# tensorboy/centerpose

Hardware: AMD Instinct MI355X
Metric: images/sec end-to-end (backbone+decode), DLA-34 512x512 (higher is better)
Workload: dtype f32

## Files before the change

### centerpose_amd/csrc/head_wino24.hip

```cpp
#include "igemm.h"

#define HW_THREADS 512
#define HW_PH 18
#define HW_PW 18
#define HW_PWP 20
#define HW_C 64
#define HW_CGS (HW_C / 4)
#define HW_CG (HW_PH * HW_PWP * 4)
#define HW_PATCH (HW_CGS * HW_CG)
#define HW_F4 (HW_PH * HW_PW * HW_CGS)
#define HW_SLOTS ((HW_F4 + HW_THREADS - 1) / HW_THREADS)
#define HW_LDR 36
#define HW_RED (16 * 32 * HW_LDR)
#define HW_LDM 36
#define HW_MID (256 * HW_LDM)
#define HW_SMEM_FLOATS (2 * HW_RED)
#define HW_SMEM_FLOATS_MM (HW_RED + HW_MID > HW_PATCH ? HW_RED + HW_MID : HW_PATCH)

typedef float hw_v2 __attribute__((ext_vector_type(2)));
typedef float hw_v4 __attribute__((ext_vector_type(4)));

struct HwHead {
    const float* w2;
    const float* b2;
    float* out2;
    int n2, ld2, act2;
};
struct HwGrid {
    int tilesX, tilesY;
    unsigned mTx, mTy;
};
__device__ __forceinline__ hw_v4 hw_lds4(const float* p) { return *reinterpret_cast<const hw_v4*>(p); }
__device__ __forceinline__ int hw_div(int n, int d, unsigned magic) { return d == 1 ? n : (int)__umulhi((unsigned)n, magic); }

__device__ __forceinline__ void hw_write_share(const f32x16 (&acc)[3], const int vh, const int P, float* wq)
{
#pragma unroll
    for (int j = 0; j < 4; ++j) {
        hw_v4 q[3];
#pragma unroll
        for (int nu = 0; nu < 3; ++nu) q[nu] = (hw_v4){acc[nu][4 * j], acc[nu][4 * j + 1], acc[nu][4 * j + 2], acc[nu][4 * j + 3]};
        hw_v4 c0, c1;
        if (vh == 0) {
            const hw_v4 s1 = q[1] + q[2], d1 = q[1] - q[2];
            c0 = P == 0 ? q[0] + s1 : s1;
            c1 = d1;
        } else {
            const hw_v4 s2 = q[0] + q[1], d2 = q[0] - q[1];
            c0 = P == 0 ? s2 : 4.f * s2;
            c1 = P == 0 ? 2.f * d2 : 8.f * d2 + q[2];
        }
        *reinterpret_cast<hw_v4*>(wq + 8 * j) = c0;
        *reinterpret_cast<hw_v4*>(wq + 32 * HW_LDR + 8 * j) = c1;
    }
}

template <int N2, int MM, bool STAG>
__global__ __launch_bounds__(HW_THREADS, 1) void head_wino24_kernel(const ConvArgs a, const HwGrid gd, const HwHead hd)
{
    static_assert(!(STAG && MM), "the second-MFMA-phase form has no staggered variant");
    extern __shared__ __attribute__((aligned(16))) float smem[];
    const int tid = threadIdx.x, lane = tid & 63, wv = __builtin_amdgcn_readfirstlane(tid >> 6);
    const int xi = wv & 3, vh = wv >> 2;
    const int h = lane >> 5, m = lane & 31;
    const int NTILES = (a.Cout + 31) >> 5;
    int t_ = ig_xcd_remap(blockIdx.x, gridDim.x), q_;
    q_ = hw_div(t_, gd.tilesX, gd.mTx); const int tx = t_ - q_ * gd.tilesX; t_ = q_;
    q_ = hw_div(t_, gd.tilesY, gd.mTy); const int ty = t_ - q_ * gd.tilesY;
    const int b = q_;
    const int y0 = ty * 16, x0 = tx * 16;
    const int ld = a.srcLd[0];
    const float* __restrict__ x = a.src[0];

    {
        float4 rg[HW_SLOTS];
        int lo[HW_SLOTS];
        bool ok[HW_SLOTS];
#pragma unroll
        for (int s = 0; s < HW_SLOTS; ++s) {
            const int idx = tid + s * HW_THREADS;
            const int pp = idx / HW_CGS, q = idx % HW_CGS;
            const int py = pp / HW_PW, px = pp - py * HW_PW;
            const int gy = y0 - 1 + py, gx = x0 - 1 + px;
            const bool inl = idx < HW_F4;
            ok[s] = inl && gy >= 0 && gy < a.H && gx >= 0 && gx < a.W;
            const int go = ok[s] ? ((b * a.H + gy) * a.W + gx) * ld + q * 4 : 0;
            lo[s] = inl ? ((q * HW_PH + py) * HW_PWP + (px ^ ((py >> 1) & 3))) * 4 : -1;
            rg[s] = ig_ldg4(x + go);
        }
#pragma unroll
        for (int s = 0; s < HW_SLOTS; ++s)
            if (lo[s] >= 0) {
                float4 v = rg[s];
                if (!ok[s]) v = make_float4(0.f, 0.f, 0.f, 0.f);
                *reinterpret_cast<float4*>(smem + lo[s]) = v;
            }
    }
    const float* up = a.w + ((size_t)xi * NTILES * (HW_C / 8)) * 1536 + (size_t)(3 * vh) * 256 + lane * 4;
    const int nlin = NTILES * (HW_C / 8);
    float4 bq[2][3];
#pragma unroll
    for (int nu = 0; nu < 3; ++nu) bq[0][nu] = ig_ldg4(up + nu * 256);
    __syncthreads();
    if constexpr (STAG) {
        if (vh == 1) __syncthreads();
    }

    const int rA = xi == 0 ? 0 : (xi == 2 ? 2 : 1);
    const int rB = xi == 2 ? 1 : (xi == 3 ? 3 : 2);
    const float sg1 = xi == 1 ? 1.f : -1.f;
    const hw_v2 sg = {sg1, sg1};
    const int tyy = m >> 2, txx = m & 3;
    const int sA = (tyy + (rA >> 1)) & 3, sB = (tyy + (rB >> 1)) & 3;
    const int baseA = ((2 * tyy + rA) * HW_PWP + 4 * txx) * 4 + h * HW_CG;
    const int baseB = ((2 * tyy + rB) * HW_PWP + 4 * txx) * 4 + h * HW_CG;
    int offA[4], offB[4];
#pragma unroll
    for (int jj = 0; jj < 4; ++jj) { offA[jj] = baseA + ((jj ^ sA) << 2); offB[jj] = baseB + ((jj ^ sB) << 2); }
    hw_v2 vl[HW_C / 8][3], vhh[HW_C / 8][3];
#pragma unroll
    for (int kc = 0; kc < HW_C / 8; ++kc) {
        const float* pc = smem + kc * 2 * HW_CG;
        hw_v2 tl[5], th[5];
        if (vh == 0) {
#pragma unroll
            for (int j = 0; j < 5; ++j) {
                const hw_v4 da = hw_lds4(pc + offA[j & 3] + (j >> 2) * 16), db = hw_lds4(pc + offB[j & 3] + (j >> 2) * 16);
                tl[j] = __builtin_elementwise_fma(sg, db.xy, da.xy);
                th[j] = __builtin_elementwise_fma(sg, db.zw, da.zw);
            }
        } else {
#pragma unroll
            for (int j = 0; j < 5; ++j) {
                const int jc = j + 1;
                const hw_v4 da = hw_lds4(pc + offA[jc & 3] + (jc >> 2) * 16), db = hw_lds4(pc + offB[jc & 3] + (jc >> 2) * 16);
                tl[j] = __builtin_elementwise_fma(sg, db.xy, da.xy);
                th[j] = __builtin_elementwise_fma(sg, db.zw, da.zw);
            }
        }
        const hw_v2 k4 = {4.f, 4.f}, kn4 = {-4.f, -4.f}, k2 = {2.f, 2.f}, kn2 = {-2.f, -2.f};
        if (vh == 0) {
            const hw_v2 al = __builtin_elementwise_fma(kn4, tl[2], tl[4]), ah = __builtin_elementwise_fma(kn4, th[2], th[4]);
            const hw_v2 bl = __builtin_elementwise_fma(kn4, tl[1], tl[3]), bh = __builtin_elementwise_fma(kn4, th[1], th[3]);
            vl[kc][0] = __builtin_elementwise_fma(k4, tl[0] - tl[2], tl[4] - tl[2]); vhh[kc][0] = __builtin_elementwise_fma(k4, th[0] - th[2], th[4] - th[2]);
            vl[kc][1] = al + bl; vhh[kc][1] = ah + bh;
            vl[kc][2] = al - bl; vhh[kc][2] = ah - bh;
        } else {
            const hw_v2 cl = tl[3] - tl[1], ch = th[3] - th[1];
            const hw_v2 fl = tl[2] - tl[0], fh = th[2] - th[0];
            vl[kc][0] = __builtin_elementwise_fma(k2, fl, cl); vhh[kc][0] = __builtin_elementwise_fma(k2, fh, ch);
            vl[kc][1] = __builtin_elementwise_fma(kn2, fl, cl); vhh[kc][1] = __builtin_elementwise_fma(kn2, fh, ch);
            vl[kc][2] = __builtin_elementwise_fma(kn4, fl, tl[4] - tl[2]); vhh[kc][2] = __builtin_elementwise_fma(kn4, fh, th[4] - th[2]);
        }
#pragma unroll
        for (int nu = 0; nu < 3; ++nu) asm volatile("" : "+v"(vl[kc][nu]), "+v"(vhh[kc][nu]));
        __builtin_amdgcn_sched_barrier(0);
    }
    if constexpr (STAG) {
        if (vh == 0) __syncthreads();
    } else {
        __syncthreads();
    }

    float acc2[2][2][N2 > 0 ? N2 : 1];
#pragma unroll
    for (int i = 0; i < 2; ++i)
#pragma unroll
        for (int k = 0; k < 2; ++k)
#pragma unroll
            for (int j = 0; j < (N2 > 0 ? N2 : 1); ++j) acc2[i][k][j] = 0.f;
    f32x16 acc2m;
#pragma unroll
    for (int r = 0; r < 16; ++r) acc2m[r] = 0.f;
    constexpr int J0 = MM ? 32 : 0;
    float* const mid = smem + HW_RED;
    const int n4 = tid & 7, bb = (tid >> 3) & 1, mi = tid >> 4;
    const int ity = mi >> 2, itx = mi & 3;
    const int itrd = (bb * 32 + mi) * HW_LDR + n4 * 4;
    const int wpo = (wv * 64 + m) * HW_LDR + 4 * h;

    int lin = 0;
    if constexpr (!MM) {
        hw_v4 sc = {0.f, 0.f, 0.f, 0.f}, sh = sc, w2r[N2];
#pragma unroll
        for (int j = 0; j < N2; ++j) w2r[j] = sc;
        hw_v4 rq[8];
        auto red_read = [&](int P) __attribute__((always_inline)) {
            int rbase = itrd + P * HW_RED;
            asm volatile("" : "+v"(rbase));
            const float* rp = smem + rbase;
#pragma unroll
            for (int w = 0; w < 8; ++w) rq[w] = hw_lds4(rp + w * 64 * HW_LDR);
        };
        auto red_sum = [&](int P) __attribute__((always_inline)) {
            const hw_v4 r0 = rq[0] + rq[4], r1 = rq[1] + rq[5], r2 = rq[2] + rq[6], r3 = rq[3] + rq[7];
            hw_v4 yv[2];
            yv[0] = (r0 + r1) + r2;
            yv[1] = (r1 - r2) - r3;
#pragma unroll
            for (int aa = 0; aa < 2; ++aa) {
                hw_v4 v = __builtin_elementwise_fma(yv[aa], sc, sh);
                v = (hw_v4){cp_relu(v.x), cp_relu(v.y), cp_relu(v.z), cp_relu(v.w)};
#pragma unroll
                for (int j = 0; j < N2; ++j) {
                    const hw_v4 w = w2r[j];
                    acc2[P][aa][j] = fmaf(v.w, w.w, fmaf(v.z, w.z, fmaf(v.y, w.y, fmaf(v.x, w.x, acc2[P][aa][j]))));
                }
            }
        };
        if constexpr (STAG) {
            auto chunk = [&](const int kc, f32x16 (&acc)[3], auto&& ride) __attribute__((always_inline)) {
                ++lin;
                const float* un = up + (size_t)(lin < nlin ? lin : nlin - 1) * 1536;
                __builtin_amdgcn_sched_barrier(0);
#pragma unroll
                for (int nu = 0; nu < 3; ++nu) {
                    if (nu == 1) {
#pragma unroll
                        for (int q = 0; q < 3; ++q) bq[(kc + 1) & 1][q] = ig_ldg4(un + q * 256);
                        __builtin_amdgcn_sched_barrier(0);
                    }
                    if (nu == 2) {
                        ride();
                        __builtin_amdgcn_sched_barrier(0);
                    }
                    const float4 bbv = bq[kc & 1][nu];
                    acc[nu] = __builtin_amdgcn_mfma_f32_32x32x2f32(bbv.x, vl[kc][nu].x, acc[nu], 0, 0, 0);
                    acc[nu] = __builtin_amdgcn_mfma_f32_32x32x2f32(bbv.y, vl[kc][nu].y, acc[nu], 0, 0, 0);
                    acc[nu] = __builtin_amdgcn_mfma_f32_32x32x2f32(bbv.z, vhh[kc][nu].x, acc[nu], 0, 0, 0);
                    acc[nu] = __builtin_amdgcn_mfma_f32_32x32x2f32(bbv.w, vhh[kc][nu].y, acc[nu], 0, 0, 0);
                }
                __builtin_amdgcn_sched_barrier(0);
            };
            auto tile_end = [&](const int nt, const f32x16 (&acc)[3], const bool barrier_first) __attribute__((always_inline)) {
                const int ncol = nt * 32 + n4 * 4;
                sc = *reinterpret_cast<const hw_v4*>(a.scale + ncol);
                sh = *reinterpret_cast<const hw_v4*>(a.shift + ncol);
#pragma unroll
                for (int j = 0; j < N2; ++j) w2r[j] = *reinterpret_cast<const hw_v4*>(hd.w2 + (size_t)j * hd.ld2 + ncol);
                if (barrier_first) __syncthreads();
#pragma unroll
                for (int P = 0; P < 2; ++P) {
                    int wbase = wpo + P * HW_RED;
                    asm volatile("" : "+v"(wbase));
                    hw_write_share(acc, vh, P, smem + wbase);
                }
            };
            const auto nothing = [] {};
            if (vh == 0) {
#pragma unroll 1
                for (int nt = 0; nt < NTILES; ++nt) {
                    const bool prev = nt > 0;
                    f32x16 acc[3];
#pragma unroll
                    for (int nu = 0; nu < 3; ++nu)
#pragma unroll
                        for (int r = 0; r < 16; ++r) acc[nu][r] = 0.f;
#pragma unroll
                    for (int kc = 0; kc < 5; ++kc) chunk(kc, acc, nothing);
                    __syncthreads();
                    chunk(5, acc, [&] { if (prev) red_read(0); });
                    chunk(6, acc, [&] { if (prev) { red_sum(0); red_read(1); } });
                    chunk(7, acc, [&] { if (prev) red_sum(1); });
                    tile_end(nt, acc, true);
                }
            } else {
#pragma unroll 1
                for (int nt = 0; nt < NTILES; ++nt) {
                    const bool prev = nt > 0;
                    f32x16 acc[3];
#pragma unroll
                    for (int nu = 0; nu < 3; ++nu)
#pragma unroll
                        for (int r = 0; r < 16; ++r) acc[nu][r] = 0.f;
                    __syncthreads();
                    chunk(0, acc, [&] { if (prev) red_read(0); });
                    chunk(1, acc, [&] { if (prev) red_sum(0); });
                    chunk(2, acc, [&] { if (prev) red_read(1); });
                    chunk(3, acc, [&] { if (prev) red_sum(1); });
                    __syncthreads();
#pragma unroll
                    for (int kc = 4; kc < 8; ++kc) chunk(kc, acc, nothing);
                    tile_end(nt, acc, false);
                }
            }
            __syncthreads();
        } else {
#pragma unroll 1
        for (int nt = 0; nt < NTILES; ++nt) {
            const bool prev = nt > 0;
            f32x16 acc[3];
#pragma unroll
            for (int nu = 0; nu < 3; ++nu)
#pragma unroll
                for (int r = 0; r < 16; ++r) acc[nu][r] = 0.f;
#pragma unroll
            for (int kc = 0; kc < HW_C / 8; ++kc) {
                ++lin;
                const float* un = up + (size_t)(lin < nlin ? lin : nlin - 1) * 1536;
                __builtin_amdgcn_sched_barrier(0);
#pragma unroll
                for (int nu = 0; nu < 3; ++nu) {
                    if (nu == 1) {
#pragma unroll
                        for (int q = 0; q < 3; ++q) bq[(kc + 1) & 1][q] = ig_ldg4(un + q * 256);
                        __builtin_amdgcn_sched_barrier(0);
                    }
                    if (nu == 2 && prev) {
                        if (kc == 0) red_read(0);
                        if (kc == 2) red_sum(0);
                        if (kc == 4) red_read(1);
                        if (kc == 6) red_sum(1);
                        __builtin_amdgcn_sched_barrier(0);
                    }
                    const float4 bbv = bq[kc & 1][nu];
                    acc[nu] = __builtin_amdgcn_mfma_f32_32x32x2f32(bbv.x, vl[kc][nu].x, acc[nu], 0, 0, 0);
                    acc[nu] = __builtin_amdgcn_mfma_f32_32x32x2f32(bbv.y, vl[kc][nu].y, acc[nu], 0, 0, 0);
                    acc[nu] = __builtin_amdgcn_mfma_f32_32x32x2f32(bbv.z, vhh[kc][nu].x, acc[nu], 0, 0, 0);
                    acc[nu] = __builtin_amdgcn_mfma_f32_32x32x2f32(bbv.w, vhh[kc][nu].y, acc[nu], 0, 0, 0);
                }
                __builtin_amdgcn_sched_barrier(0);
            }
            const int ncol = nt * 32 + n4 * 4;
            sc = *reinterpret_cast<const hw_v4*>(a.scale + ncol);
            sh = *reinterpret_cast<const hw_v4*>(a.shift + ncol);
#pragma unroll
            for (int j = 0; j < N2; ++j) w2r[j] = *reinterpret_cast<const hw_v4*>(hd.w2 + (size_t)j * hd.ld2 + ncol);
            if (prev) __syncthreads();
#pragma unroll
            for (int P = 0; P < 2; ++P) {
                int wbase = wpo + P * HW_RED;
                asm volatile("" : "+v"(wbase));
                float* wq = smem + wbase;
#pragma unroll
                for (int j = 0; j < 4; ++j) {
                    hw_v4 q[3];
#pragma unroll
                    for (int nu = 0; nu < 3; ++nu) q[nu] = (hw_v4){acc[nu][4 * j], acc[nu][4 * j + 1], acc[nu][4 * j + 2], acc[nu][4 * j + 3]};
                    hw_v4 c0, c1;
                    if (vh == 0) {
                        const hw_v4 s1 = q[1] + q[2], d1 = q[1] - q[2];
                        c0 = P == 0 ? q[0] + s1 : s1;
                        c1 = d1;
                    } else {
                        const hw_v4 s2 = q[0] + q[1], d2 = q[0] - q[1];
                        c0 = P == 0 ? s2 : 4.f * s2;
                        c1 = P == 0 ? 2.f * d2 : 8.f * d2 + q[2];
                    }
                    *reinterpret_cast<hw_v4*>(wq + 8 * j) = c0;
                    *reinterpret_cast<hw_v4*>(wq + 32 * HW_LDR + 8 * j) = c1;
                }
            }
            __syncthreads();
        }
        }
        red_read(0); red_sum(0);
        red_read(1); red_sum(1);
    } else {
#pragma unroll 1
    for (int nt = 0; nt < NTILES; ++nt) {
        f32x16 acc[3];
#pragma unroll
        for (int nu = 0; nu < 3; ++nu)
#pragma unroll
            for (int r = 0; r < 16; ++r) acc[nu][r] = 0.f;
#pragma unroll
        for (int kc = 0; kc < HW_C / 8; ++kc) {
            ++lin;
            const float* un = up + (size_t)(lin < nlin ? lin : nlin - 1) * 1536;
            __builtin_amdgcn_sched_barrier(0);
#pragma unroll
            for (int nu = 0; nu < 3; ++nu) {
                if (nu == 1) {
#pragma unroll
                    for (int q = 0; q < 3; ++q) bq[(kc + 1) & 1][q] = ig_ldg4(un + q * 256);
                    __builtin_amdgcn_sched_barrier(0);
                }
                const float4 bbv = bq[kc & 1][nu];
                acc[nu] = __builtin_amdgcn_mfma_f32_32x32x2f32(bbv.x, vl[kc][nu].x, acc[nu], 0, 0, 0);
                acc[nu] = __builtin_amdgcn_mfma_f32_32x32x2f32(bbv.y, vl[kc][nu].y, acc[nu], 0, 0, 0);
                acc[nu] = __builtin_amdgcn_mfma_f32_32x32x2f32(bbv.z, vhh[kc][nu].x, acc[nu], 0, 0, 0);
                acc[nu] = __builtin_amdgcn_mfma_f32_32x32x2f32(bbv.w, vhh[kc][nu].y, acc[nu], 0, 0, 0);
            }
            __builtin_amdgcn_sched_barrier(0);
        }

        const int ncol = nt * 32 + n4 * 4;
        const hw_v4 sc = *reinterpret_cast<const hw_v4*>(a.scale + ncol), sh = *reinterpret_cast<const hw_v4*>(a.shift + ncol);
        hw_v4 w2r[N2 > 0 ? N2 : 1];
#pragma unroll
        for (int j = 0; j < N2; ++j) w2r[j] = *reinterpret_cast<const hw_v4*>(hd.w2 + (size_t)(J0 + j) * hd.ld2 + ncol);
        hw_v4 w2f[MM ? 4 : 1];
#pragma unroll
        for (int P = 0; P < 2; ++P) {
            if (MM && P == 1) __syncthreads();
            int wbase = wpo + (MM ? 0 : P * HW_RED), rbase = itrd + (MM ? 0 : P * HW_RED);
            asm volatile("" : "+v"(wbase), "+v"(rbase));
            float* wq = smem + wbase;
#pragma unroll
            for (int j = 0; j < 4; ++j) {
                hw_v4 q[3];
#pragma unroll
                for (int nu = 0; nu < 3; ++nu) q[nu] = (hw_v4){acc[nu][4 * j], acc[nu][4 * j + 1], acc[nu][4 * j + 2], acc[nu][4 * j + 3]};
                hw_v4 c0, c1;
                if (vh == 0) {
                    const hw_v4 s1 = q[1] + q[2], d1 = q[1] - q[2];
                    c0 = P == 0 ? q[0] + s1 : s1;
                    c1 = d1;
                } else {
                    const hw_v4 s2 = q[0] + q[1], d2 = q[0] - q[1];
                    c0 = P == 0 ? s2 : 4.f * s2;
                    c1 = P == 0 ? 2.f * d2 : 8.f * d2 + q[2];
                }
                *reinterpret_cast<hw_v4*>(wq + 8 * j) = c0;
                *reinterpret_cast<hw_v4*>(wq + 32 * HW_LDR + 8 * j) = c1;
            }
            if constexpr (MM) {
                if (P == 1) {
                    const int nmm = hd.n2 < 32 ? hd.n2 : 32;
                    const bool live = m < nmm;
                    const float* wrow = hd.w2 + (size_t)(live ? m : nmm - 1) * hd.ld2 + nt * 32 + 4 * h;
#pragma unroll
                    for (int s4 = 0; s4 < 4; ++s4) {
                        const float4 t4 = ig_ldg4(wrow + 8 * s4);
                        w2f[s4] = live ? (hw_v4){t4.x, t4.y, t4.z, t4.w} : (hw_v4){0.f, 0.f, 0.f, 0.f};
                    }
                }
            }
            __syncthreads();
            const float* rp = smem + rbase;
            hw_v4 r0 = hw_lds4(rp) + hw_lds4(rp + 4 * 64 * HW_LDR);
            const hw_v4 r1 = hw_lds4(rp + 64 * HW_LDR) + hw_lds4(rp + 5 * 64 * HW_LDR);
            const hw_v4 r2 = hw_lds4(rp + 2 * 64 * HW_LDR) + hw_lds4(rp + 6 * 64 * HW_LDR);
            const hw_v4 r3 = hw_lds4(rp + 3 * 64 * HW_LDR) + hw_lds4(rp + 7 * 64 * HW_LDR);
            hw_v4 yv[2];
            yv[0] = (r0 + r1) + r2;
            yv[1] = (r1 - r2) - r3;
#pragma unroll
            for (int aa = 0; aa < 2; ++aa) {
                hw_v4 v = __builtin_elementwise_fma(yv[aa], sc, sh);
                v = (hw_v4){cp_relu(v.x), cp_relu(v.y), cp_relu(v.z), cp_relu(v.w)};
#pragma unroll
                for (int j = 0; j < N2; ++j) {
                    const hw_v4 w = w2r[j];
                    acc2[P][aa][j] = fmaf(v.w, w.w, fmaf(v.z, w.z, fmaf(v.y, w.y, fmaf(v.x, w.x, acc2[P][aa][j]))));
                }
                if constexpr (MM) {
                    *reinterpret_cast<hw_v4*>(mid + ((2 * ity + aa) * 16 + 4 * itx + 2 * P + bb) * HW_LDM + n4 * 4) = v;
                }
            }
        }
        if constexpr (MM) {
            __syncthreads();
            const float* mp = mid + (32 * wv + m) * HW_LDM + 4 * h;
            hw_v4 mf[4];
#pragma unroll
            for (int s4 = 0; s4 < 4; ++s4) mf[s4] = hw_lds4(mp + 8 * s4);
#pragma unroll
            for (int s4 = 0; s4 < 4; ++s4) {
                acc2m = __builtin_amdgcn_mfma_f32_32x32x2f32(w2f[s4].x, mf[s4].x, acc2m, 0, 0, 0);
                acc2m = __builtin_amdgcn_mfma_f32_32x32x2f32(w2f[s4].y, mf[s4].y, acc2m, 0, 0, 0);
                acc2m = __builtin_amdgcn_mfma_f32_32x32x2f32(w2f[s4].z, mf[s4].z, acc2m, 0, 0, 0);
                acc2m = __builtin_amdgcn_mfma_f32_32x32x2f32(w2f[s4].w, mf[s4].w, acc2m, 0, 0, 0);
            }
            __syncthreads();
        }
    }

    }
    const size_t HW = (size_t)a.H * a.W;
    if constexpr (MM) {
        const int p = 32 * wv + m, ox = x0 + (p & 15), oy = y0 + (p >> 4);
        const int nmm = hd.n2 < 32 ? hd.n2 : 32;
        if (ox < a.W && oy < a.H) {
#pragma unroll
            for (int r = 0; r < 16; ++r) {
                const int j = (r & 3) + 8 * (r >> 2) + 4 * h;
                if (j < nmm) hd.out2[((size_t)b * hd.n2 + j) * HW + (size_t)oy * a.W + ox] = cp_act(acc2m[r] + hd.b2[j], hd.act2);
            }
        }
    }
    if constexpr (N2 > 0) {
#pragma unroll
        for (int P = 0; P < 2; ++P) {
            const int ox = x0 + 4 * itx + 2 * P + bb, oy = y0 + 2 * ity;
#pragma unroll
            for (int aa = 0; aa < 2; ++aa)
#pragma unroll
                for (int j = 0; j < N2; ++j) {
                    float v = acc2[P][aa][j];
                    v += __shfl_xor(v, 1);
                    v += __shfl_xor(v, 2);
                    v += __shfl_xor(v, 4);
                    if ((tid & 7) == 0 && J0 + j < hd.n2 && ox < a.W && oy + aa < a.H)
                        hd.out2[((size_t)b * hd.n2 + J0 + j) * HW + (size_t)(oy + aa) * a.W + ox] = cp_act(v + hd.b2[J0 + j], hd.act2);
                }
        }
    }
}

static unsigned hw_magic(int d) { return d <= 1 ? 0u : (unsigned)(((1ull << 32) + (unsigned)d - 1) / (unsigned)d); }

template <int N2, int MM, bool STAG = false>
static int launch_head_wino24(const ConvArgs& a, hipStream_t s, const HwHead& hd)
{
    const int smem = (MM ? HW_SMEM_FLOATS_MM : HW_SMEM_FLOATS) * 4;
    static CpLdsGuard guard;
    {
        const hipError_t e = guard.ensure((const void*)head_wino24_kernel<N2, MM, STAG>, smem);
        if (e != hipSuccess) { cp_set_error("head_wino24: cannot reserve %d B LDS: %s", smem, hipGetErrorString(e)); return 2; }
    }
    HwGrid gd;
    gd.tilesX = cp_cdiv(a.W, 16); gd.tilesY = cp_cdiv(a.H, 16);
    gd.mTx = hw_magic(gd.tilesX); gd.mTy = hw_magic(gd.tilesY);
    const long long grid = (long long)a.B * gd.tilesX * gd.tilesY;
    const long long dmax = gd.tilesX > gd.tilesY ? gd.tilesX : gd.tilesY;
    if (grid * dmax >= (1ll << 32)) { cp_set_error("head_wino24: grid %lld too large", grid); return 1; }
    hipLaunchKernelGGL((head_wino24_kernel<N2, MM, STAG>), dim3((unsigned)grid), dim3(HW_THREADS), smem, s, a, gd, hd);
    cp_note_kernel("head_wino24_kernel<%d, %d>", N2, MM);
    return 0;
}

int cp_launch_head3x3_1x1_w24(const ConvArgs& a, const float* w2, const float* b2, float* out2, int n2, int ld2, int act2, hipStream_t s)
{
    const bool ok = a.nsrc == 1 && a.kh == 3 && a.kw == 3 && a.sy == 1 && a.sx == 1 && a.py == 1 && a.px == 1 && a.Ho == a.H &&
                    a.Wo == a.W && a.srcC[0] == 64 && a.srcLd[0] % 4 == 0 && a.Cout % 32 == 0 && a.act == CP_ACT_RELU && !a.res &&
                    n2 >= 1 && n2 <= 34 && ld2 % 4 == 0 && ld2 >= a.Cout &&
                    (((size_t)a.src[0] | (size_t)a.w | (size_t)w2 | (size_t)a.scale | (size_t)a.shift) & 15) == 0 &&
                    (long long)a.B * a.H * a.W * a.srcLd[0] < (1ll << 31);
    if (!ok) return -1;
    HwHead hd;
    hd.w2 = w2; hd.b2 = b2; hd.out2 = out2; hd.n2 = n2; hd.ld2 = ld2; hd.act2 = act2;
    const char* sw = getenv("CP_HEAD_STAGGER");
    const bool stag = !(sw && sw[0] == '0');
    if (n2 == 1) return stag ? launch_head_wino24<1, 0, true>(a, s, hd) : launch_head_wino24<1, 0>(a, s, hd);
    if (n2 == 2) return stag ? launch_head_wino24<2, 0, true>(a, s, hd) : launch_head_wino24<2, 0>(a, s, hd);
    if (n2 <= 32) return launch_head_wino24<0, 1>(a, s, hd);
    if (n2 == 33) return launch_head_wino24<1, 1>(a, s, hd);
    return launch_head_wino24<2, 1>(a, s, hd);
}
```

### centerpose_amd/ops.py

```python
import ctypes
import os

import torch

from . import _lib

ACT_NONE, ACT_RELU, ACT_SIGMOID, ACT_HSWISH, ACT_HSIGMOID = 0, 1, 2, 3, 4
BN_EPS = 1e-5


class ConvDesc(ctypes.Structure):
    _fields_ = [(n, ctypes.c_int) for n in ("nsrc",)] + [("srcC", ctypes.c_int * 4), ("srcLd", ctypes.c_int * 4)] + \
        [(n, ctypes.c_int) for n in ("B", "H", "W", "Ho", "Wo", "kh", "kw", "sy", "sx", "py", "px", "K", "ldw", "Cout",
                                     "resLd", "outLd", "outNCHW", "OH", "OW", "osy", "osx", "ooy", "oox", "act",
                                     "inNCHW", "tile", "nsub", "ksplit")]


class DcnDesc(ctypes.Structure):
    _fields_ = [(n, ctypes.c_int) for n in ("B", "H", "W", "C", "srcLd", "Ho", "Wo", "kh", "kw", "sy", "sx", "py", "px",
                                            "dily", "dilx", "K", "ldw", "Cout", "omLd", "omSigmoid", "outLd",
                                            "outNCHW", "act", "tile", "ksplit", "dg")]


def round_up(x, m):
# ... 154 lines not shown


BATCH_INVARIANT = os.environ.get("CP_BATCH_INVARIANT", "0") == "1"


def rule_batch(B):
    return 1 if BATCH_INVARIANT else B


SPLIT_BF16 = os.environ.get("CP_SPLIT_BF16", "0") == "1"
SPLIT_BF16_TILES = ((128, 128), (128, 64), (64, 128), (64, 64))


def split_bf16_weight(wp, ldw):
    L = _lib.lib()
    rows, K = wp.shape
    assert rows % ldw == 0 and K % 16 == 0 and wp.is_contiguous()
    L.cp_split_bf16_weight_floats.restype = ctypes.c_size_t
    wb = torch.empty((L.cp_split_bf16_weight_floats(rows, K),), dtype=torch.float32, device=wp.device)
    _lib.check(L.cp_split_bf16_weights_f32(_lib.ptr(wp), rows, ldw, K, _lib.ptr(wb), _lib.stream()), "cp_split_bf16_weights_f32")
    return wb


def split_bf16_tile(M, ldw, nsub=1, ksplit=1, force=False, K=None):
    if ldw % 64:
        return None
    code = lambda bm, bn: 3000000 + bm * 1000 + bn
    forced = os.environ.get("CP_SPLIT_BF16_TILE")
    if forced:
        bm, bn = (int(v) for v in forced.split("x")) if "x" in forced else (128, int(forced))
        return code(bm, bn if ldw % bn == 0 else 64)
    blocks = lambda bm, bn: ((M + bm - 1) // bm) * max(1, nsub) * max(1, ksplit) * (ldw // bn)
    floor = 0 if force else int(os.environ.get("CP_SPLIT_BF16_MINBLOCKS", "512"))
    if floor == 0:
        return code(128, 128) if ldw % 128 == 0 and blocks(128, 128) >= 256 else code(128, 64)
    if ksplit > 1:
        return None
    order = ((64, 64),) if K is not None and K <= 64 else ((128, 128), (64, 128), (64, 64))
    for bm, bn in order:
        if ldw % bn == 0 and blocks(bm, bn) >= floor:
            return code(bm, bn)
    return None


def conv2d(srcs, wp, scale, shift, out, **kw):
    conv2d_launch(srcs, wp, scale, shift, out, **kw).run()
    return out


def conv2d_launch(srcs, wp, scale, shift, out, *, kh, kw, stride=1, pad=0, cout, act=ACT_NONE, res=None, out_nchw=False,
                  in_nchw=False, Ho=None, Wo=None, pad_yx=None, out_scatter=None, tile=0, wino=None, nsub=1, ksplit=0, split_bf16=None):
    d = ConvDesc()
    d.nsrc = len(srcs)
    if in_nchw:
        x = srcs[0]
        B, C, H, W = x.shape
        d.srcC[0], d.srcLd[0] = C, 0
        assert B * C * H * W < 2 ** 31, "conv2d: NCHW source of %d floats exceeds the 32-bit element index of the stem producers" % (B * C * H * W)
        assert x.is_contiguous()
    else:
        B, H, W, _ = srcs[0].shape
        for i, s in enumerate(srcs):
            assert s.shape[:3] == srcs[0].shape[:3]
            d.srcC[i], d.srcLd[i] = s.shape[3], _ld(s)
    py, px = pad_yx if pad_yx is not None else (pad, pad)
    if Ho is None:
        Ho = (H + 2 * py - kh) // stride + 1
        Wo = (W + 2 * px - kw) // stride + 1
    assert B * Ho * Wo + 255 < 2 ** 31, "conv2d: B*Ho*Wo=%d output pixels exceed the 32-bit row index" % (B * Ho * Wo)
    d.B, d.H, d.W, d.Ho, d.Wo = B, H, W, Ho, Wo
    d.kh, d.kw, d.sy, d.sx, d.py, d.px = kh, kw, stride, stride, py, px
    assert wp.shape[0] % nsub == 0
    d.K, d.ldw, d.Cout, d.nsub = wp.shape[1], wp.shape[0] // nsub, cout, nsub
    d.resLd = _ld(res) if res is not None else 0
    d.outNCHW = 1 if out_nchw else 0
    d.ksplit = ksplit
    if ksplit > 1:
        assert res is None and act == ACT_NONE and not out_nchw and out.is_contiguous() and (wino is not None or (len(srcs) == 1 and not in_nchw and nsub == 1))
        assert tuple(out.shape[:2]) == (ksplit, B * Ho * Wo) and out.shape[2] >= cout and out.shape[2] % 4 == 0
        d.OH, d.OW, d.outLd = Ho, Wo, out.shape[2]
    elif out_nchw:
        d.OH, d.OW, d.outLd = out.shape[2], out.shape[3], 0
        assert out.is_contiguous() and out.shape[1] == cout
    else:
        d.OH, d.OW, d.outLd = out.shape[1], out.shape[2], _ld(out)
    d.osy, d.osx, d.ooy, d.oox = out_scatter if out_scatter is not None else (1, 1, 0, 0)
    d.act, d.inNCHW, d.tile = act, 1 if in_nchw else 0, tile
    for t in (wp, scale, shift, wino):
        assert t is None or t.is_contiguous()
    if wino is not None:
        assert len(srcs) == 1 and not in_nchw
        return Launch("cp_conv3x3_winograd_f32", d, [srcs[0], wino, scale, shift, res, out])
    if (SPLIT_BF16 if split_bf16 is None else split_bf16) and tile == 0 and not in_nchw:
        code = split_bf16_tile(rule_batch(B) * Ho * Wo, d.ldw, nsub, ksplit, force=split_bf16 is True, K=d.K)
        c16 = kh == 3 and kw == 3 and len(srcs) == 1 and srcs[0].shape[3] == 16 and cout <= 32
        if code is not None and not c16 and all(s.data_ptr() % 16 == 0 for s in srcs):
            d.tile = code
            wp = split_bf16_weight(wp, d.ldw)
    return Launch("cp_conv2d_f32", d, list(srcs) + [None] * (4 - len(srcs)) + [wp, scale, shift, res, out])


ConvDesc4 = ConvDesc * 4


def conv3x3_group_launch(members, whole):
    assert 1 <= len(members) <= 4
    members = sorted(members, key=lambda mm: -mm["x"].shape[3])
    d = ConvDesc4()
    cols = [[None] * 4 for _ in range(6)]
    for i, mm in enumerate(members):
        one = conv2d_launch([mm["x"]], mm["wp"], mm["scale"], mm["shift"], mm["out"], kh=3, kw=3, stride=1, pad=1, cout=mm["cout"],
                            act=mm["act"], res=mm["res"], wino=mm["u24"], tile=WINO24)
        ctypes.memmove(ctypes.addressof(d[i]), ctypes.addressof(one.desc), ctypes.sizeof(ConvDesc))
        for k, t in enumerate((mm["x"], mm["u24"], mm["scale"], mm["shift"], mm["res"], mm["out"])):
            cols[k][i] = t
            assert t is None or k in (0, 4, 5) or t.is_contiguous()
        assert mm["out"].untyped_storage().data_ptr() == whole.untyped_storage().data_ptr()
    return Launch("cp_conv3x3_winograd24_group_f32", d, [t for col in cols for t in col] + [whole], [len(members)])


ConvDesc8 = ConvDesc * 8
GROUP_MAX = 8


def conv2d_group_launch(members, whole):
    assert 1 <= len(members) <= GROUP_MAX
    members = sorted(members, key=lambda mm: -mm["wp"].shape[1])
    d = ConvDesc8()
    cols = [[None] * GROUP_MAX for _ in range(6)]
    for i, mm in enumerate(members):
        assert mm["wp"].shape[0] % 64 == 0
        one = conv2d_launch([mm["x"]], mm["wp"], mm["scale"], mm["shift"], mm["out"], kh=mm["k"], kw=mm["k"], stride=mm["stride"],
                            pad=mm["pad"], cout=mm["cout"], act=mm["act"], res=mm.get("res"), split_bf16=False)
        ctypes.memmove(ctypes.addressof(d[i]), ctypes.addressof(one.desc), ctypes.sizeof(ConvDesc))
        for k, t in enumerate((mm["x"], mm["wp"], mm["scale"], mm["shift"], mm.get("res"), mm["out"])):
            cols[k][i] = t
            assert t is None or k in (0, 4, 5) or t.is_contiguous()
        assert mm["out"].untyped_storage().data_ptr() == whole.untyped_storage().data_ptr()
    return Launch("cp_conv2d_group_f32", d, [t for col in cols for t in col] + [whole], [len(members)])


def head3x3_1x1_eligible(x, hc, n2):
    B, H, W, C = x.shape
    B = rule_batch(B)
    return C == 64 and hc % 32 == 0 and hc >= 128 and 1 <= n2 <= 34 and B * ((H + 7) // 8) * ((W + 15) // 16) >= 512


def head_wino24_wanted(x, n2):
    B, H, W, _ = x.shape
    B = rule_batch(B)
    mode = os.environ.get("CP_HEAD24", "1")
    if mode == "0" or B * ((H + 15) // 16) * ((W + 15) // 16) < 256:
        return False
    return mode == "all" or n2 <= 32


def head3x3_1x1_launch(x, u, scale, shift, w2, b2, out2, *, hc, act2=ACT_NONE, wino24=False):
    B, H, W, C = x.shape
    n2, ld2 = w2.shape
    assert out2.is_contiguous() and tuple(out2.shape) == (B, n2, H, W) and w2.is_contiguous() and b2.numel() >= n2
    d = ConvDesc()
    d.nsrc = 1
    d.srcC[0], d.srcLd[0] = C, _ld(x)
    d.B, d.H, d.W, d.Ho, d.Wo = B, H, W, H, W
    d.kh, d.kw, d.sy, d.sx, d.py, d.px = 3, 3, 1, 1, 1, 1
    d.K, d.ldw, d.Cout = 9 * C, round_up(hc, 64), hc
    d.resLd, d.outLd, d.outNCHW = 0, hc, 0
    d.OH, d.OW, d.osy, d.osx, d.ooy, d.oox = H, W, 1, 1, 0, 0
    d.act, d.inNCHW, d.tile, d.nsub = ACT_RELU, 0, WINO24 if wino24 else 0, 1
    return Launch("cp_head3x3_1x1_f32", d, [x, u, scale, shift, w2, b2, out2], [n2, ld2, act2])


def wino_eligible(cin, k, stride, pad, nsrc=1):
    return k == 3 and stride == 1 and pad == 1 and nsrc == 1 and cin % 16 == 0 and cin >= 32


def pack_wino_weight(wp, cin, cout):
    L = _lib.lib()
    assert wp.shape[1] == 9 * cin and wp.shape[0] >= cout and wp.is_contiguous()
    L.cp_winograd_weight_floats.restype = ctypes.c_size_t
    n = L.cp_winograd_weight_floats(cin, cout)
    assert n > 0, "winograd: C must be a multiple of 16"
    u = torch.empty((n,), dtype=torch.float32, device=wp.device)
    _lib.check(L.cp_winograd_pack_f32(_lib.ptr(wp), _lib.ptr(u), cin, cout, _lib.stream()), "cp_winograd_pack_f32")
    return u


def pack_wino24_weight(wp, cin, cout):
    L = _lib.lib()
    assert wp.shape[1] == 9 * cin and wp.shape[0] >= cout and wp.is_contiguous()
    L.cp_winograd24_weight_floats.restype = ctypes.c_size_t
    n = L.cp_winograd24_weight_floats(cin, cout)
    assert n > 0, "winograd: C must be a multiple of 16"
    u = torch.empty((n,), dtype=torch.float32, device=wp.device)
    _lib.check(L.cp_winograd24_pack_f32(_lib.ptr(wp), _lib.ptr(u), cin, cout, _lib.stream()), "cp_winograd24_pack_f32")
    return u


WINO24 = 24


def wino24_wanted(B, H, W, cin, cout):
    if os.environ.get("CP_WINO24", "1") == "0" or cin % 16 or cin < 32:
        return False
    minc, mincout, minblocks = (int(v) for v in os.environ.get("CP_WINO24_RULE", "32,16,256").split(","))
    blocks = rule_batch(B) * ((H + 15) // 16) * ((W + 15) // 16) * ((cout + 31) // 32)
    return cin >= minc and cout >= mincout and blocks >= minblocks


def dcn_v2(x, om, wp, scale, shift, out, **kw):
    dcn_v2_launch(x, om, wp, scale, shift, out, **kw).run()
    return out


def _pair(v):
    return (int(v[0]), int(v[1])) if isinstance(v, (tuple, list)) else (int(v), int(v))


def dcn_v2_launch(x, om, wp, scale, shift, out, *, cout, kh=3, kw=3, stride=1, pad=1, dil=1, om_sigmoid=True,
                  act=ACT_NONE, out_nchw=False, tile=0, ksplit=0, dg=1):
    B, H, W, C = x.shape
    d = DcnDesc()
    (sy, sx), (py, px), (dy, dx) = _pair(stride), _pair(pad), _pair(dil)
    Ho = (H + 2 * py - (dy * (kh - 1) + 1)) // sy + 1
    Wo = (W + 2 * px - (dx * (kw - 1) + 1)) // sx + 1
    assert om.shape[:3] == (B, Ho, Wo)
    d.B, d.H, d.W, d.C, d.srcLd, d.Ho, d.Wo = B, H, W, C, _ld(x), Ho, Wo
    d.kh, d.kw, d.sy, d.sx, d.py, d.px, d.dily, d.dilx = kh, kw, sy, sx, py, px, dy, dx
    d.K, d.ldw, d.Cout = wp.shape[1], wp.shape[0], cout
    d.omLd, d.omSigmoid = _ld(om), 1 if om_sigmoid else 0
    d.outNCHW = 1 if out_nchw else 0
    d.act, d.tile, d.ksplit, d.dg = act, tile, ksplit, dg
    if ksplit > 1:
        assert tuple(out.shape) == (ksplit, B * Ho * Wo, wp.shape[0]) and out.is_contiguous() and cout == wp.shape[0] and act == ACT_NONE
        d.outLd = wp.shape[0]
    else:
        d.outLd = 0 if out_nchw else _ld(out)
    return Launch("cp_dcn_v2_f32", d, [x, om, wp, scale, shift, out])


def wino_ksplit(B, H, W, cin, cout):
    blocks = rule_batch(B) * ((H + 7) // 8) * ((W + 15) // 16) * ((cout + 31) // 32)
    stages = cin // 16
    S = 1
    while blocks * S < 512 and stages // (2 * S) >= 4:
        S *= 2
    return S if blocks < 256 else 1


def conv_ksplit(M, ldw, K):
    if ldw % 64 != 0:
        return 1
    blocks = ((M + 63) // 64) * (ldw // 64)
    if blocks >= 400:
        return 1
    for S in (2, 3, 4):
        if blocks * S >= 512 and (K // 16) // S >= 16:
            return S
    return 1


def dcn_ksplit(M, ldw, taps=9):
    if ldw % 64 != 0 or taps < 3:
        return 1
    blocks = -(-M // 64) * (ldw // 64)
    return 3 if blocks < 512 else 1


def splitk_reduce_launch(ws, scale, shift, out, *, cout, act=ACT_NONE):
    S, M, ldw = ws.shape
    assert ws.is_contiguous() and out.shape[0] * out.shape[1] * out.shape[2] == M and scale.numel() >= ldw and shift.numel() >= ldw
    return Launch("cp_splitk_reduce_f32", None, [ws, scale, shift, out], [S, M, ldw, act, _ld(out), cout])


def maxpool2d_launch(x, out, k, s, p):
    B, H, W, C = x.shape
    return Launch("cp_maxpool2d_nhwc_f32", None, [x, out], [_ld(x), _ld(out), B, H, W, C, k, s, p])


def maxpool2d(x, out, k, s, p):
    maxpool2d_launch(x, out, k, s, p).run()
    return out


def pack_dw_deconv_weight(w):
    C, _, k, _ = w.shape
    return w.reshape(C, k * k).t().contiguous().float()


def dw_deconv_add_launch(x, wk, add, out, f):
    B, H, W, C = x.shape
    assert wk.is_contiguous()
    return Launch("cp_dw_deconv_add_nhwc_f32", None, [x, wk, add, out],
                  [_ld(x), _ld(add) if add is not None else 0, _ld(out), B, H, W, C, f])


def dw_deconv_add(x, wk, add, out, f):
    dw_deconv_add_launch(x, wk, add, out, f).run()
    return out


def pack_dw_weight(w):
    C, _, k, _ = w.shape
    return w.reshape(C, k * k).t().contiguous().float()


def dwconv2d_launch(x, wk, scale, shift, out, k, stride, pad, act=ACT_NONE):
# ... 214 lines not shown
```

Before: 2255.

## Add staggered two-group schedule for MFMA-phase Winograd head kernels and enable by default

Adds a staggered variant of the fused 3x3+1x1 Winograd head kernel for the second-MFMA-phase (n2>2) forms: the two wave groups run offset tile schedules, so one group's reduction, mid-tile write and 1x1 MFMA phase overlap the other group's main MFMA chunks. For n2==34, per-thread partial sums are parked in LDS to save registers. Wino24 is also enabled by default for heads with n2>32. This adds barriers and LDS traffic, and register pressure may still be a risk.

```diff
diff --git a/centerpose_amd/csrc/head_wino24.hip b/centerpose_amd/csrc/head_wino24.hip
--- a/centerpose_amd/csrc/head_wino24.hip
+++ b/centerpose_amd/csrc/head_wino24.hip
@@ -1,5 +1,9 @@
 #include "igemm.h"
-
+#include <type_traits>
+
+#ifndef HW_SETPRIO
+#define HW_SETPRIO 0
+#endif
 #define HW_THREADS 512
 #define HW_PH 18
 #define HW_PW 18
@@ -16,6 +20,8 @@
 #define HW_MID (256 * HW_LDM)
 #define HW_SMEM_FLOATS (2 * HW_RED)
 #define HW_SMEM_FLOATS_MM (HW_RED + HW_MID > HW_PATCH ? HW_RED + HW_MID : HW_PATCH)
+#define HW_PARK(N2, MM, STAG) ((N2) == 2 && (MM) && (STAG))
+#define HW_SMEM_FLOATS_PARK (2 * HW_RED + HW_THREADS * 8)
 
 typedef float hw_v2 __attribute__((ext_vector_type(2)));
 typedef float hw_v4 __attribute__((ext_vector_type(4)));
@@ -55,10 +61,36 @@
     }
 }
 
+template <class Ride>
+__device__ __forceinline__ void hw_chunk(const int kc, f32x16 (&acc)[3], float4 (&bq)[2][3], const hw_v2 (&vl)[HW_C / 8][3],
+                                         const hw_v2 (&vhh)[HW_C / 8][3], const float* up, int& lin, const int nlin, Ride&& ride)
+{
+    ++lin;
+    const float* un = up + (size_t)(lin < nlin ? lin : nlin - 1) * 1536;
+    __builtin_amdgcn_sched_barrier(0);
+#pragma unroll
+    for (int nu = 0; nu < 3; ++nu) {
+        if (nu == 1) {
+#pragma unroll
+            for (int q = 0; q < 3; ++q) bq[(kc + 1) & 1][q] = ig_ldg4(un + q * 256);
+            __builtin_amdgcn_sched_barrier(0);
+        }
+        if (nu == 2) {
+            ride();
+            __builtin_amdgcn_sched_barrier(0);
+        }
+        const float4 bbv = bq[kc & 1][nu];
+        acc[nu] = __builtin_amdgcn_mfma_f32_32x32x2f32(bbv.x, vl[kc][nu].x, acc[nu], 0, 0, 0);
+        acc[nu] = __builtin_amdgcn_mfma_f32_32x32x2f32(bbv.y, vl[kc][nu].y, acc[nu], 0, 0, 0);
+        acc[nu] = __builtin_amdgcn_mfma_f32_32x32x2f32(bbv.z, vhh[kc][nu].x, acc[nu], 0, 0, 0);
+        acc[nu] = __builtin_amdgcn_mfma_f32_32x32x2f32(bbv.w, vhh[kc][nu].y, acc[nu], 0, 0, 0);
+    }
+    __builtin_amdgcn_sched_barrier(0);
+}
+
 template <int N2, int MM, bool STAG>
 __global__ __launch_bounds__(HW_THREADS, 1) void head_wino24_kernel(const ConvArgs a, const HwGrid gd, const HwHead hd)
 {
-    static_assert(!(STAG && MM), "the second-MFMA-phase form has no staggered variant");
     extern __shared__ __attribute__((aligned(16))) float smem[];
     const int tid = threadIdx.x, lane = tid & 63, wv = __builtin_amdgcn_readfirstlane(tid >> 6);
     const int xi = wv & 3, vh = wv >> 2;
@@ -180,6 +212,7 @@
     const int wpo = (wv * 64 + m) * HW_LDR + 4 * h;
 
     int lin = 0;
+    int te = tid;
     if constexpr (!MM) {
         hw_v4 sc = {0.f, 0.f, 0.f, 0.f}, sh = sc, w2r[N2];
 #pragma unroll
@@ -210,27 +243,7 @@
         };
         if constexpr (STAG) {
             auto chunk = [&](const int kc, f32x16 (&acc)[3], auto&& ride) __attribute__((always_inline)) {
-                ++lin;
-                const float* un = up + (size_t)(lin < nlin ? lin : nlin - 1) * 1536;
-                __builtin_amdgcn_sched_barrier(0);
-#pragma unroll
-                for (int nu = 0; nu < 3; ++nu) {
-                    if (nu == 1) {
-#pragma unroll
-                        for (int q = 0; q < 3; ++q) bq[(kc + 1) & 1][q] = ig_ldg4(un + q * 256);
-                        __builtin_amdgcn_sched_barrier(0);
-                    }
-                    if (nu == 2) {
-                        ride();
-                        __builtin_amdgcn_sched_barrier(0);
-                    }
-                    const float4 bbv = bq[kc & 1][nu];
-                    acc[nu] = __builtin_amdgcn_mfma_f32_32x32x2f32(bbv.x, vl[kc][nu].x, acc[nu], 0, 0, 0);
-                    acc[nu] = __builtin_amdgcn_mfma_f32_32x32x2f32(bbv.y, vl[kc][nu].y, acc[nu], 0, 0, 0);
-                    acc[nu] = __builtin_amdgcn_mfma_f32_32x32x2f32(bbv.z, vhh[kc][nu].x, acc[nu], 0, 0, 0);
-                    acc[nu] = __builtin_amdgcn_mfma_f32_32x32x2f32(bbv.w, vhh[kc][nu].y, acc[nu], 0, 0, 0);
-                }
-                __builtin_amdgcn_sched_barrier(0);
+                hw_chunk(kc, acc, bq, vl, vhh, up, lin, nlin, ride);
             };
             auto tile_end = [&](const int nt, const f32x16 (&acc)[3], const bool barrier_first) __attribute__((always_inline)) {
                 const int ncol = nt * 32 + n4 * 4;
@@ -265,6 +278,9 @@
                     tile_end(nt, acc, true);
                 }
             } else {
+#if HW_SETPRIO
+                __builtin_amdgcn_s_setprio(1);
+#endif
 #pragma unroll 1
                 for (int nt = 0; nt < NTILES; ++nt) {
                     const bool prev = nt > 0;
@@ -356,6 +372,208 @@
         }
         red_read(0); red_sum(0);
         red_read(1); red_sum(1);
+    } else if constexpr (STAG) {
+        constexpr bool PARK = HW_PARK(N2, MM, STAG);
+        constexpr int NR = N2 > 0 ? N2 : 1;
+        hw_v4 sc, sh, w2r[NR], w2f[4], rq[4], r01[2], vm[2], mf[4];
+        const int nmm = hd.n2 < 32 ? hd.n2 : 32;
+        int o_rd, o_wp, o_mw, o_mp;
+        int o_a2;
+        unsigned wro, cbo;
+        bool live;
+        auto own_offsets = [&]() __attribute__((always_inline)) {
+            int t = tid;
+            asm volatile("" : "+v"(t));
+            const int tm = t & 31, th = (t >> 5) & 1, t4 = t & 7, tb = (t >> 3) & 1, ti = t >> 4;
+            o_rd = (tb * 32 + ti) * HW_LDR + t4 * 4;
+            o_wp = (wv * 64 + tm) * HW_LDR + 4 * th;
+            o_mw = (2 * (ti >> 2) * 16 + 4 * (ti & 3) + tb) * HW_LDM + t4 * 4;
+            o_mp = (32 * wv + tm) * HW_LDM + 4 * th;
+            live = tm < nmm;
+            wro = (unsigned)(((live ? tm : nmm - 1) * hd.ld2 + 4 * th) * 4);
+            cbo = (unsigned)(t4 * 16);
+            o_a2 = 2 * HW_RED + t * 8;
+            asm volatile("" : "+v"(o_a2));
+        };
+        auto gld = [](const float* base, const unsigned byteoff) __attribute__((always_inline)) {
+            asm volatile("" : "+s"(base));
+            return *(const __attribute__((address_space(1))) hw_v4*)(reinterpret_cast<const char*>(base) + byteoff);
+        };
+        auto cols_load = [&](const int pt) __attribute__((always_inline)) {
+            sc = gld(a.scale + pt * 32, cbo);
+            sh = gld(a.shift + pt * 32, cbo);
+#pragma unroll
+            for (int j = 0; j < N2; ++j) w2r[j] = gld(hd.w2 + (size_t)(J0 + j) * hd.ld2 + pt * 32, cbo);
+        };
+        auto w2f_load = [&](const int pt) __attribute__((always_inline)) {
+#pragma unroll
+            for (int s4 = 0; s4 < 4; ++s4) {
+                const hw_v4 t4 = gld(hd.w2 + pt * 32 + 8 * s4, wro);
+                w2f[s4] = live ? t4 : (hw_v4){0.f, 0.f, 0.f, 0.f};
+            }
+        };
+        auto red_read = [&](const int P) __attribute__((always_inline)) {
+            int rbase = o_rd + P * HW_RED;
+            asm volatile("" : "+v"(rbase));
+            const float* rp = smem + rbase;
+            rq[0] = hw_lds4(rp);                  rq[1] = hw_lds4(rp + 4 * 64 * HW_LDR);
+            rq[2] = hw_lds4(rp + 64 * HW_LDR);    rq[3] = hw_lds4(rp + 5 * 64 * HW_LDR);
+            r01[0] = rq[0] + rq[1];
+            r01[1] = rq[2] + rq[3];
+            __builtin_amdgcn_sched_barrier(0);
+            rq[0] = hw_lds4(rp + 2 * 64 * HW_LDR); rq[1] = hw_lds4(rp + 6 * 64 * HW_LDR);
+            rq[2] = hw_lds4(rp + 3 * 64 * HW_LDR); rq[3] = hw_lds4(rp + 7 * 64 * HW_LDR);
+        };
+        auto red_vals = [&](const int P) __attribute__((always_inline)) {
+            const hw_v4 r0 = r01[0], r1 = r01[1], r2 = rq[0] + rq[1], r3 = rq[2] + rq[3];
+            hw_v4 yv[2];
+            yv[0] = (r0 + r1) + r2;
+            yv[1] = (r1 - r2) - r3;
+#pragma unroll
+            for (int aa = 0; aa < 2; ++aa) {
+                hw_v4 v = __builtin_elementwise_fma(yv[aa], sc, sh);
+                v = (hw_v4){cp_relu(v.x), cp_relu(v.y), cp_relu(v.z), cp_relu(v.w)};
+#pragma unroll
+                for (int j = 0; j < N2; ++j) {
+                    const hw_v4 w = w2r[j];
+                    float* const park = smem + o_a2 + (P * 2 + aa) * N2 + j;
+                    const float s0 = PARK ? *park : acc2[P][aa][j];
+                    const float s1 = fmaf(v.w, w.w, fmaf(v.z, w.z, fmaf(v.y, w.y, fmaf(v.x, w.x, s0))));
+                    if constexpr (PARK) *park = s1;
+                    else acc2[P][aa][j] = s1;
+                }
+                vm[aa] = v;
+            }
+        };
+        auto mid_write = [&](const int P) __attribute__((always_inline)) {
+#pragma unroll
+            for (int aa = 0; aa < 2; ++aa) *reinterpret_cast<hw_v4*>(smem + o_mw + (aa * 16 + 2 * P) * HW_LDM) = vm[aa];
+        };
+        auto mid_read = [&]() __attribute__((always_inline)) {
+#pragma unroll
+            for (int s4 = 0; s4 < 4; ++s4) mf[s4] = hw_lds4(smem + o_mp + 8 * s4);
+        };
+        auto phase2 = [&]() __attribute__((always_inline)) {
+#pragma unroll
+            for (int s4 = 0; s4 < 4; ++s4) {
+                acc2m = __builtin_amdgcn_mfma_f32_32x32x2f32(w2f[s4].x, mf[s4].x, acc2m, 0, 0, 0);
+                acc2m = __builtin_amdgcn_mfma_f32_32x32x2f32(w2f[s4].y, mf[s4].y, acc2m, 0, 0, 0);
+                acc2m = __builtin_amdgcn_mfma_f32_32x32x2f32(w2f[s4].z, mf[s4].z, acc2m, 0, 0, 0);
+                acc2m = __builtin_amdgcn_mfma_f32_32x32x2f32(w2f[s4].w, mf[s4].w, acc2m, 0, 0, 0);
+            }
+        };
+        auto write_shares = [&](const f32x16 (&acc)[3]) __attribute__((always_inline)) {
+#pragma unroll
+            for (int P = 0; P < 2; ++P) {
+                int wbase = o_wp + P * HW_RED;
+                asm volatile("" : "+v"(wbase));
+                hw_write_share(acc, vh, P, smem + wbase);
+            }
+        };
+        auto chunk = [&](float4 (&bl)[2][3], const int kc, f32x16 (&acc)[3], auto&& ride) __attribute__((always_inline)) {
+            hw_chunk(kc, acc, bl, vl, vhh, up, lin, nlin, ride);
+        };
+        auto zero_sums = [&]() __attribute__((always_inline)) {
+#pragma unroll
+            for (int i = 0; i < 2; ++i)
+#pragma unroll
+                for (int k = 0; k < 2; ++k)
+#pragma unroll
+                    for (int j = 0; j < NR; ++j) {
+                        if constexpr (PARK) smem[o_a2 + (i * 2 + k) * N2 + j] = 0.f;
+                        else acc2[i][k][j] = 0.f;
+                    }
+#pragma unroll
+            for (int r = 0; r < 16; ++r) acc2m[r] = 0.f;
+        };
+        const auto nothing = [] {};
+        auto tile_a = [&](float4 (&bl)[2][3], const int nt, auto prev_c) __attribute__((always_inline)) {
+            constexpr bool PREV = decltype(prev_c)::value;
+            if constexpr (!PREV) { own_offsets(); zero_sums(); }
+            f32x16 acc[3];
+#pragma unroll
+            for (int nu = 0; nu < 3; ++nu)
+#pragma unroll
+                for (int r = 0; r < 16; ++r) acc[nu][r] = 0.f;
+#pragma unroll
+            for (int kc = 0; kc < 5; ++kc) chunk(bl, kc, acc, nothing);
+            __syncthreads();
+            chunk(bl, 5, acc, [&] { if constexpr (PREV) { cols_load(nt - 1); red_read(0); } });
+            chunk(bl, 6, acc, [&] { if constexpr (PREV) { red_vals(0); red_read(1); } });
+            __syncthreads();
+            chunk(bl, 7, acc, [&] { if constexpr (PREV) { mid_write(0); red_vals(1); mid_write(1); w2f_load(nt - 1); } });
+            __syncthreads();
+            if constexpr (PREV) { mid_read(); phase2(); }
+            __builtin_amdgcn_sched_barrier(0);
+            __syncthreads();
+            write_shares(acc);
+        };
+        auto tile_b = [&](float4 (&bl)[2][3], const int nt, auto prev_c) __attribute__((always_inline)) {
+            constexpr bool PREV = decltype(prev_c)::value;
+            if constexpr (!PREV) { own_offsets(); zero_sums(); }
+            f32x16 acc[3];
+#pragma unroll
+            for (int nu = 0; nu < 3; ++nu)
+#pragma unroll
+                for (int r = 0; r < 16; ++r) acc[nu][r] = 0.f;
+            if constexpr (!PREV) {
+                const float* upb = up;
+                asm volatile("" : "+v"(upb));
+#pragma unroll
+                for (int nu = 0; nu < 3; ++nu) bl[0][nu] = ig_ldg4(upb + nu * 256);
+            }
+            __syncthreads();
+            chunk(bl, 0, acc, [&] { if constexpr (PREV) { cols_load(nt - 1); red_read(0); } });
+            chunk(bl, 1, acc, [&] { if constexpr (PREV) { red_vals(0); red_read(1); } });
+            __syncthreads();
+            chunk(bl, 2, acc, [&] { if constexpr (PREV) { mid_write(0); red_vals(1); mid_write(1); w2f_load(nt - 1); } });
+            __syncthreads();
+            chunk(bl, 3, acc, [&] { if constexpr (PREV) mid_read(); });
+            if constexpr (PREV) phase2();
+            __builtin_amdgcn_sched_barrier(0);
+            __syncthreads();
+#pragma unroll
+            for (int kc = 4; kc < 8; ++kc) chunk(bl, kc, acc, nothing);
+            write_shares(acc);
+        };
+        int grp = vh;
+        asm volatile("" : "+s"(grp));
+        if (grp == 1) {
+            float4 bl[2][3];
+#if HW_SETPRIO
+            __builtin_amdgcn_s_setprio(1);
+#endif
+            tile_b(bl, 0, std::false_type{});
+#pragma unroll 1
+            for (int nt = 1; nt < NTILES; ++nt) tile_b(bl, nt, std::true_type{});
+        } else {
+            float4 bl[2][3];
+#pragma unroll
+            for (int nu = 0; nu < 3; ++nu) bl[0][nu] = bq[0][nu];
+            tile_a(bl, 0, std::false_type{});
+#pragma unroll 1
+            for (int nt = 1; nt < NTILES; ++nt) tile_a(bl, nt, std::true_type{});
+        }
+        __syncthreads();
+        int last = NTILES - 1;
+        own_offsets();
+        asm volatile("" : "+s"(last));
+        cols_load(last);
+        w2f_load(last);
+        red_read(0); red_vals(0); red_read(1);
+        __syncthreads();
+        mid_write(0); red_vals(1); mid_write(1);
+        __syncthreads();
+        mid_read(); phase2();
+        if constexpr (PARK) {
+            te = (o_a2 - 2 * HW_RED) >> 3;
+#pragma unroll
+            for (int i = 0; i < 2; ++i)
+#pragma unroll
+                for (int k = 0; k < 2; ++k)
+#pragma unroll
+                    for (int j = 0; j < N2; ++j) acc2[i][k][j] = smem[o_a2 + (i * 2 + k) * N2 + j];
+        }
     } else {
 #pragma unroll 1
     for (int nt = 0; nt < NTILES; ++nt) {
@@ -469,13 +687,16 @@
 
     }
     const size_t HW = (size_t)a.H * a.W;
+    constexpr bool PK = HW_PARK(N2, MM, STAG);
+    const int e_m = PK ? te & 31 : m, e_h = PK ? (te >> 5) & 1 : h, e_bb = PK ? (te >> 3) & 1 : bb, e_ity = PK ? te >> 6 : ity,
+              e_itx = PK ? (te >> 4) & 3 : itx, e_t = PK ? te : tid;
     if constexpr (MM) {
-        const int p = 32 * wv + m, ox = x0 + (p & 15), oy = y0 + (p >> 4);
+        const int p = 32 * wv + e_m, ox = x0 + (p & 15), oy = y0 + (p >> 4);
         const int nmm = hd.n2 < 32 ? hd.n2 : 32;
         if (ox < a.W && oy < a.H) {
 #pragma unroll
             for (int r = 0; r < 16; ++r) {
-                const int j = (r & 3) + 8 * (r >> 2) + 4 * h;
+                const int j = (r & 3) + 8 * (r >> 2) + 4 * e_h;
                 if (j < nmm) hd.out2[((size_t)b * hd.n2 + j) * HW + (size_t)oy * a.W + ox] = cp_act(acc2m[r] + hd.b2[j], hd.act2);
             }
         }
@@ -483,7 +704,7 @@
     if constexpr (N2 > 0) {
 #pragma unroll
         for (int P = 0; P < 2; ++P) {
-            const int ox = x0 + 4 * itx + 2 * P + bb, oy = y0 + 2 * ity;
+            const int ox = x0 + 4 * e_itx + 2 * P + e_bb, oy = y0 + 2 * e_ity;
 #pragma unroll
             for (int aa = 0; aa < 2; ++aa)
 #pragma unroll
@@ -492,7 +713,7 @@
                     v += __shfl_xor(v, 1);
                     v += __shfl_xor(v, 2);
                     v += __shfl_xor(v, 4);
-                    if ((tid & 7) == 0 && J0 + j < hd.n2 && ox < a.W && oy + aa < a.H)
+                    if ((e_t & 7) == 0 && J0 + j < hd.n2 && ox < a.W && oy + aa < a.H)
                         hd.out2[((size_t)b * hd.n2 + J0 + j) * HW + (size_t)(oy + aa) * a.W + ox] = cp_act(v + hd.b2[J0 + j], hd.act2);
                 }
         }
@@ -504,7 +725,7 @@
 template <int N2, int MM, bool STAG = false>
 static int launch_head_wino24(const ConvArgs& a, hipStream_t s, const HwHead& hd)
 {
-    const int smem = (MM ? HW_SMEM_FLOATS_MM : HW_SMEM_FLOATS) * 4;
+    const int smem = (HW_PARK(N2, MM, STAG) ? HW_SMEM_FLOATS_PARK : MM && !STAG ? HW_SMEM_FLOATS_MM : HW_SMEM_FLOATS) * 4;
     static CpLdsGuard guard;
     {
         const hipError_t e = guard.ensure((const void*)head_wino24_kernel<N2, MM, STAG>, smem);
@@ -535,7 +756,7 @@
     const bool stag = !(sw && sw[0] == '0');
     if (n2 == 1) return stag ? launch_head_wino24<1, 0, true>(a, s, hd) : launch_head_wino24<1, 0>(a, s, hd);
     if (n2 == 2) return stag ? launch_head_wino24<2, 0, true>(a, s, hd) : launch_head_wino24<2, 0>(a, s, hd);
-    if (n2 <= 32) return launch_head_wino24<0, 1>(a, s, hd);
-    if (n2 == 33) return launch_head_wino24<1, 1>(a, s, hd);
-    return launch_head_wino24<2, 1>(a, s, hd);
+    if (n2 <= 32) return stag ? launch_head_wino24<0, 1, true>(a, s, hd) : launch_head_wino24<0, 1>(a, s, hd);
+    if (n2 == 33) return stag ? launch_head_wino24<1, 1, true>(a, s, hd) : launch_head_wino24<1, 1>(a, s, hd);
+    return stag ? launch_head_wino24<2, 1, true>(a, s, hd) : launch_head_wino24<2, 1>(a, s, hd);
 }
diff --git a/centerpose_amd/ops.py b/centerpose_amd/ops.py
--- a/centerpose_amd/ops.py
+++ b/centerpose_amd/ops.py
@@ -330,7 +330,7 @@
     mode = os.environ.get("CP_HEAD24", "1")
     if mode == "0" or B * ((H + 15) // 16) * ((W + 15) // 16) < 256:
         return False
-    return mode == "all" or n2 <= 32
+    return mode != "32" or n2 <= 32
 
 
 def head3x3_1x1_launch(x, u, scale, shift, w2, b2, out2, *, hc, act2=ACT_NONE, wino24=False):
```

Result: no change. 2258, median of 2 (+0.1%).
